# ami-iit/paper_gorbani_2025_humanoids_multi-rate-mpc-ironcub

Hardware: AMD Instinct MI355X
Metric: MPC solves/sec (whole node) + p50 single-solve latency, iRonCub paper horizon (higher is better)
Workload: dtype f64

## Files before the change

### paper_gorbani_2025_humanoids_multi-rate-mpc-ironcub_amd/csrc/vsmpc_p4.hpp

```cpp
#pragma once
#include "vsmpc_smem.hpp"

namespace vsmpc {

template <int K, int NVS>
VS_DEV double small_spd_solve(const double* __restrict__ sP, unsigned long long mask, double rhs, int lane, int& bad) {
    int idx[K];
#pragma unroll
    for (int q = 0; q < K; ++q) {
        idx[q] = __ffsll((long long)mask) - 1;
        mask &= mask - 1;
    }
    double A[K][K], d[K];
#pragma unroll
    for (int q = 0; q < K; ++q) {
        d[q] = readlane_f64(rhs, idx[q]);
#pragma unroll
        for (int c = 0; c <= q; ++c) A[q][c] = sP[idx[c] * NVS + idx[q]];
    }
    double ip[K];
#pragma unroll
    for (int j = 0; j < K; ++j) {
        bad |= !(A[j][j] > 0.0);
        ip[j] = fast_rcp(A[j][j]);
#pragma unroll
        for (int i = j + 1; i < K; ++i) {
            const double f = A[i][j] * ip[j];
            d[i] = fma(-f, d[j], d[i]);
#pragma unroll
            for (int c = j + 1; c <= i; ++c) A[i][c] = fma(-f, A[c][j], A[i][c]);
        }
    }
    double x[K], mu = 0.0;
#pragma unroll
    for (int j = K - 1; j >= 0; --j) {
        double t = d[j];
#pragma unroll
        for (int c = j + 1; c < K; ++c) t = fma(-A[c][j], x[c], t);
        x[j] = t * ip[j];
        mu = (lane == idx[j]) ? x[j] : mu;
    }
    return mu;
}

constexpr int SMALL_SOLVE_MAX = 6;
constexpr int AS_PATIENCE = 10;
constexpr int AS_MAX_ITER = 64;
template <int NVS, int K = SMALL_SOLVE_MAX>
VS_DEV double small_spd_solve_n(int k, const double* __restrict__ sP, unsigned long long mask, double rhs, int lane, int& bad) {
    if constexpr (K == 1) {
        return small_spd_solve<1, NVS>(sP, mask, rhs, lane, bad);
    } else {
        if (k == K) return small_spd_solve<K, NVS>(sP, mask, rhs, lane, bad);
        return small_spd_solve_n<NVS, K - 1>(k, sP, mask, rhs, lane, bad);
    }
}

template <class D>
VS_DEV void schur_rhs(const double* __restrict__ Lb, double* __restrict__ sSvec, int lane) {
    constexpr int PV = D::NU >> 4;
    constexpr int GR = D::NZ - 16 * (PV + 1);
    const int r = lane < D::NV ? lane : D::NV - 1;
    const double* L76 = Lb + tile_off<D>(PV + 1, PV);
    const double* L77 = Lb + tile_off<D>(PV + 1, PV + 1);
    const double* rowp = Lb + tile_off<D>(PV + (r >> 4), PV) + (r & 15) * 17;
    double sr = 0.0;
#pragma unroll
    for (int c = 0; c < D::NV; ++c) {
        const double lrc = rowp[((c >> 4) && (r >> 4)) ? D::TS + (c & 15) : (c & 15)];
        const double ellc = c < 16 ? L76[GR * 17 + c] : L77[GR * 17 + (c - 16)];
        sr = fma(c <= r ? lrc : 0.0, ellc, sr);
    }
    if (lane < D::NV) sSvec[r] = sr;
}

template <class D>
struct XTiles {
    static constexpr int NVS = D::NV + 1, NR2 = D::NV - 16;
    static constexpr int KMAX = SMALL_SOLVE_MAX;
    static constexpr int KMID = 16;
    const double* X6;
    const double* sXr;
    VS_DEV double col(int j, int r, int n) const {
        const double t = j < 16 ? X6[j * 17 + (r & 15)] : sXr[(j - 16) * NVS + r];
        return (j < 16 ? r < 16 : j < n) ? t : 0.0;
    }
    VS_DEV double pcol(int b, int r, int n) const {
        double p0 = 0.0, p1 = 0.0;
        if (b < 16) {
#pragma unroll
            for (int j = 0; j < 16; j += 2) {
                p0 = fma(col(j, r, n), X6[j * 17 + b], p0);
                p1 = fma(col(j + 1, r, n), X6[(j + 1) * 17 + b], p1);
            }
        }
#pragma unroll
        for (int a2 = 0; a2 < NR2; ++a2) p0 = fma(col(16 + a2, r, n), sXr[a2 * NVS + b], p0);
        return p0 + p1;
    }
};
template <class D>
struct XDense {
    static constexpr int NVS = D::NV + 1;
    static constexpr int KMAX = 10;
    static constexpr int KMID = 24;
    const double* sXd;
    VS_DEV double col(int j, int r, int n) const { return j < n ? sXd[j * NVS + r] : 0.0; }
    VS_DEV double pcol(int b, int r, int n) const {
        double p0 = 0.0, p1 = 0.0;
        int j = b;
        for (; j + 1 < n; j += 2) {
            p0 = fma(sXd[j * NVS + r], sXd[j * NVS + b], p0);
            p1 = fma(sXd[(j + 1) * NVS + r], sXd[(j + 1) * NVS + b], p1);
        }
        if (j < n) p0 = fma(sXd[j * NVS + r], sXd[j * NVS + b], p0);
        return p0 + p1;
    }
};

template <int KMID, int NVS>
VS_DEV double mid_spd_solve(int ka, const double* __restrict__ sP, unsigned long long Amask, double bb, int lane, bool isA,
                            int& bad) {
    int idx[KMID];
    {
        unsigned long long m = Amask;
#pragma unroll
        for (int q = 0; q < KMID; ++q) {
            idx[q] = m ? __ffsll((long long)m) - 1 : 0;
            m &= m - 1;
        }
    }
    const int rank = __popcll(Amask & ((1ull << lane) - 1ull));
    double a[KMID];
#pragma unroll
    for (int q = 0; q < KMID; ++q) a[q] = sP[idx[q] * NVS + lane];
#pragma unroll
    for (int j = 0; j < KMID; ++j) {
        if (j < ka) {
            const double piv = readlane_f64(a[j], idx[j]);
            bad |= !(piv > 0.0);
            const double ip = fast_rcp(piv);
            const double bj = readlane_f64(bb, idx[j]);
            const double f = (isA && rank > j) ? a[j] * ip : 0.0;
            bb = fma(-f, bj, bb);
#pragma unroll
            for (int c = j + 1; c < KMID; ++c) {
                if (c < ka) {
                    const double pc = readlane_f64(a[c], idx[j]);
                    a[c] = fma(-f, pc, a[c]);
                }
            }
        }
    }
    double mu = 0.0;
#pragma unroll
    for (int j = KMID - 1; j >= 0; --j) {
        if (j < ka) {
            const double xj = readlane_f64(bb, idx[j]) * fast_rcp(readlane_f64(a[j], idx[j]));
            mu = (lane == idx[j]) ? xj : mu;
            bb = (isA && rank < j) ? fma(-a[j], xj, bb) : bb;
        }
    }
    return mu;
}

template <class D, class XA>
VS_DEV void dual_active_set(const XA& xa, bool hold, int lane, double* __restrict__ sSv, double* __restrict__ sQP,
                            const double* __restrict__ sSvec, const double* __restrict__ sVprev,
                            const double* __restrict__ sCfg, double* __restrict__ sZ, int* __restrict__ sFlags,
                            unsigned long long have0 = 0ull) {
    constexpr int NVS = D::NV + 1;
    double* sP = sSv;
    double* sK = sQP;
    const int r = lane < D::NV ? lane : D::NV - 1;
    const bool valid = lane < D::NV;
    const bool fixed = valid && hold && (r >= D::NV - 4);
    const int n = hold ? D::NV - 4 : D::NV;
    const bool inN = valid && r < n;
    const double lo = fixed ? sVprev[r & 3] : sCfg[CFG_VMIN];
    const double hi = fixed ? sVprev[r & 3] : sCfg[CFG_VMAX];
    const double gtol = 1e-10 * (1.0 + sSvec[0]);
    const double vu = sZ[D::NU + r];
    int state = 0;
    double v = vu;
    int best, patience = AS_PATIENCE, status = VSMPC_STATUS_MAX_ITER, iters = 1, bad = 0;
    {
        const double tolv = 1e-12 * (1.0 + fabs(v));
        const bool vlo = inN && (v < lo - tolv);
        const bool vhi = inN && (v > hi + tolv);
        best = __popcll(__ballot(vlo || vhi));
        if (vlo || vhi) state = vlo ? -1 : 1;
    }
    unsigned long long have = have0;
    for (int it = 1; it < AS_MAX_ITER; ++it) {
        iters = it + 1;
        const bool isA = inN && state != 0;
        const unsigned long long Amask = __ballot(isA);
        unsigned long long need = Amask & ~have;
        have |= need;
        while (need) {
            const int b = __ffsll((long long)need) - 1;
            need &= need - 1;
            const double pb = xa.pcol(b, r, n);
            if (valid) sP[b * NVS + r] = pb;
        }
        double bb = isA ? vu - (state < 0 ? lo : hi) : 0.0;
        double mu = 0.0;
        const int ka = __popcll(Amask);
        if (ka == 0) {
        } else if (ka <= XA::KMAX) {
            mu = small_spd_solve_n<D::NV + 1, XA::KMAX>(ka, sP, Amask, bb, lane, bad);
        } else if (XA::KMID > 0 && ka <= XA::KMID) {
            if constexpr (XA::KMID > 0) mu = mid_spd_solve<XA::KMID, D::NV + 1>(ka, sP, Amask, bb, lane, isA, bad);
        } else {
            if (isA) {
                unsigned long long m = Amask;
                while (m) {
                    const int c = __ffsll((long long)m) - 1;
                    m &= m - 1;
                    sK[r * NVS + c] = sP[c * NVS + r];
                }
            }
            for (unsigned long long pm = Amask; pm; pm &= pm - 1) {
                const int j = __ffsll((long long)pm) - 1;
                const double piv = sK[j * NVS + j];
                bad |= !(piv > 0.0);
                const double bj = readlane_f64(bb, j);
                if (isA && lane > j) {
                    const double f = sK[r * NVS + j] * fast_rcp(piv);
                    bb -= f * bj;
                    for (unsigned long long m = pm & (pm - 1); m; m &= m - 1) {
                        const int c = __ffsll((long long)m) - 1;
                        sK[r * NVS + c] -= f * sK[j * NVS + c];
                    }
                }
            }
            for (unsigned long long pm = Amask; pm;) {
                const int j = 63 - __clzll((long long)pm);
                pm &= ~(1ull << j);
                const double xj = readlane_f64(bb, j) * fast_rcp(sK[j * NVS + j]);
                if (lane == j) mu = xj;
                if (isA && lane < j) bb -= sK[r * NVS + j] * xj;
            }
        }
        if (bad) { status = VSMPC_STATUS_NUMERICAL; break; }
        v = vu;
        for (unsigned long long m = Amask; m; m &= m - 1) {
            const int b = __ffsll((long long)m) - 1;
            const double mub = readlane_f64(mu, b);
            if (inN) v -= sP[b * NVS + r] * mub;
        }
        const double grad = -mu;
        const double tolv = 1e-12 * (1.0 + fabs(v));
        const bool isF = inN && state == 0;
        const bool vlo = isF && (v < lo - tolv);
        const bool vhi = isF && (v > hi + tolv);
        const bool rlo = isA && state == -1 && grad < -gtol;
        const bool rhi = isA && state == 1 && grad > gtol;
        const bool inf = vlo || vhi || rlo || rhi;
        const unsigned long long imask = __ballot(inf);
        const int ninf = __popcll(imask);
        if (ninf == 0) { status = VSMPC_STATUS_SOLVED; break; }
        bool pick = inf;
        if (ninf < best) { best = ninf; patience = AS_PATIENCE; }
        else if (patience > 0) { --patience; }
        else { pick = inf && (lane == 63 - __clzll(imask)); }
        if (pick) state = vlo ? -1 : (vhi ? 1 : 0);
    }
    if (valid) {
        v = fixed ? lo : (state < 0 ? lo : (state > 0 ? hi : v));
        sZ[D::NU + lane] = v;
    }
    if (lane == 0) { sFlags[1] = status; sFlags[2] = iters; }
}

template <class D>
VS_DEV void box_qp(int n_violated, bool hold, int wave) {
    using S = Smem<D>;
    extern __shared__ __attribute__((aligned(16))) double smem[];
    double* sVprev = smem + S::oVprev;
    double* sInvD = smem + S::oInvD;
    double* sZ = smem + S::oZ;
    double* sSv = smem + S::oSv;
    double* sSvec = smem + S::oSvec;
    double* sCfg = smem + S::oCfg;
    int* sFlags = reinterpret_cast<int*>(smem + S::oFlags);
    double* Lb = smem + S::oM;
    double* sXinv = smem + S::oXinv;
    double* sQP = smem + S::oQP;
    const int lane = fresh_lane(), tid = (wave << 6) | lane;
    constexpr bool DUALQP = S::DUALQP;
    constexpr int PV = D::PVT;
    constexpr int DUAL_MAX_ACTIVE = 16;
    constexpr bool DUAL3 = S::DUAL3;
    constexpr int DUAL3_MAX = 24;
    const bool few = n_violated <= (DUAL3 ? DUAL3_MAX : DUAL_MAX_ACTIVE);
    (void)sQP; (void)sXinv; (void)sInvD;
      if (few && DUALQP) {
       if constexpr (DUALQP) {
        {
            constexpr int NVS = D::NV + 1, NR2 = D::NV - 16;
            double* sXr = sQP + D::NV * NVS;
            double* sT = sQP;
            const double* X6 = sXinv + PV * D::TS;
            const double* L76 = Lb + tile_off<D>(PV + 1, PV);
            const double* L77 = Lb + tile_off<D>(PV + 1, PV + 1);
            constexpr int XT0 = 17 * NR2 <= 192 ? 16 * NR2 : 224;
            static_assert(XT0 + NR2 <= D::BLOCK && D::NV <= 32, "threads of the X77 columns");
            if (tid < 16 * NR2) {
                const int a2 = tid >> 4, j = tid & 15;
                double t0 = 0.0, t1 = 0.0;
#pragma unroll
                for (int k = 0; k < 16; k += 2) {
                    t0 = fma(L76[a2 * 17 + k], X6[k * 17 + j], t0);
                    t1 = fma(L76[a2 * 17 + k + 1], X6[(k + 1) * 17 + j], t1);
                }
                sT[a2 * 16 + j] = t0 + t1;
            } else if (tid >= XT0 && tid < XT0 + NR2) {
                const int c = tid - XT0;
                double x[NR2];
#pragma unroll
                for (int i = 0; i < NR2; ++i) {
                    double sum = 0.0;
#pragma unroll
                    for (int k = 0; k < i; ++k) sum = fma(L77[i * 17 + k], (k >= c) ? x[k] : 0.0, sum);
                    const double di = sInvD[D::NU + 16 + i];
                    x[i] = (i == c) ? di : ((i > c) ? -di * sum : 0.0);
                    sXr[i * NVS + 16 + c] = x[i];
                }
            } else if (wave == 3) {
                schur_rhs<D>(Lb, sSvec, lane);
            }
            __syncthreads();
            if (wave == 3) {
                double gm = 0.0;
#pragma unroll
                for (int c = 0; c < D::NV; ++c) gm = fmax(gm, fabs(sSvec[c]));
                if (lane == 0) sSvec[0] = gm;
            }
            if (tid < 16 * NR2) {
                const int a2 = tid >> 4, j = tid & 15;
                double t = 0.0;
#pragma unroll
                for (int b2 = 0; b2 < NR2; ++b2) t = fma(sXr[a2 * NVS + 16 + b2], sT[b2 * 16 + j], t);
                sXr[a2 * NVS + j] = -t;
            }
            __syncthreads();
        }
        static_assert(D::NU % 16 == 0 && D::NV > 16 && D::NV <= 32, "throttle block: tile aligned, two tile rows");
        const XTiles<D> xa{sXinv + PV * D::TS, sQP + D::NV * (D::NV + 1)};
        const bool all_cols = n_violated > 4;
        if (all_cols) {
            const int n = hold ? D::NV - 4 : D::NV;
            for (int e = tid; e < D::NV * D::NV; e += D::BLOCK) {
                const int b = e / D::NV, r = e - b * D::NV;
                sSv[b * (D::NV + 1) + r] = xa.pcol(b, r, n);
            }
            __syncthreads();
        }
        if (wave == 0)
            dual_active_set<D>(xa, hold, lane, sSv, sQP, sSvec, sVprev, sCfg, sZ, sFlags, all_cols ? ((1ull << D::NV) - 1ull) : 0ull);
       }
      } else if (few && DUAL3) {
       if constexpr (DUAL3) {
        constexpr int NVS = D::NV + 1, R2 = D::NV - 32;
        double* sXd = sQP + D::NV * NVS;
        double* sT0 = smem + S::oDual3T0;
        double* sT1 = smem + S::oDual3T1;
        static_assert(S::oDual3T0 == S::oQP + 2 * D::NV * NVS, "scratch tiles behind K and X");
        const double* L10 = Lb + tile_off<D>(PV + 1, PV);
        const double* L20 = Lb + tile_off<D>(PV + 2, PV);
        const double* L21 = Lb + tile_off<D>(PV + 2, PV + 1);
        const double* X0 = sXinv + PV * D::TS;
        auto xd = [&](int blk_r, int blk_c) { return sXd + (16 * blk_r) * NVS + 16 * blk_c; };
        for (int e = tid; e < D::NV * NVS; e += D::BLOCK) sXd[e] = 0.0;
        if (tid < 4 * D::NV) {
            const int i = tid >> 2, part = tid & 3;
            double sum = 0.0;
            for (int k = part; k <= i; k += 4)
                sum += Lb[lower_at<D>(D::NU + i, D::NU + k)] * Lb[lower_at<D>(D::NZ, D::NU + k)];
            sSv[tid] = sum;
        }
        __syncthreads();
        {
            const int g = lane >> 4, n = lane & 15;
            auto a_tile = [&](const double* T, int ks) { return T[n * 17 + 4 * ks + g]; };
            auto b_tile = [&](const double* T, int ks) { return T[(4 * ks + g) * 17 + n]; };
            auto a_x2 = [&](int ks) {
                const double v = sT1[n * 17 + 4 * ks + g];
                return (n < R2 && 4 * ks + g < R2) ? v : 0.0;
            };
            const d4 zero = d4{0.0, 0.0, 0.0, 0.0};
            if (wave == 0) {
                d4 t10 = zero, x10 = zero, t20 = zero, x20 = zero;
#pragma unroll
                for (int ks = 0; ks < 4; ++ks) t10 = __builtin_amdgcn_mfma_f64_16x16x4f64(a_tile(L10, ks), b_tile(X0, ks), t10, 0, 0, 0);
#pragma unroll
                for (int ks = 0; ks < 4; ++ks) t20 = __builtin_amdgcn_mfma_f64_16x16x4f64(a_tile(L20, ks), b_tile(X0, ks), t20, 0, 0, 0);
#pragma unroll
                for (int ks = 0; ks < 4; ++ks) x10 = __builtin_amdgcn_mfma_f64_16x16x4f64(a_tile(sT0, ks), t10[ks], x10, 0, 0, 0);
#pragma unroll
                for (int r = 0; r < 4; ++r) { x10[r] = -x10[r]; xd(1, 0)[(g + 4 * r) * NVS + n] = x10[r]; }
#pragma unroll
                for (int ks = 0; ks < 4; ++ks) t20 = __builtin_amdgcn_mfma_f64_16x16x4f64(a_tile(L21, ks), x10[ks], t20, 0, 0, 0);
#pragma unroll
                for (int ks = 0; ks < 4; ++ks) x20 = __builtin_amdgcn_mfma_f64_16x16x4f64(a_x2(ks), t20[ks], x20, 0, 0, 0);
#pragma unroll
                for (int r = 0; r < 4; ++r)
                    if (g + 4 * r < R2) xd(2, 0)[(g + 4 * r) * NVS + n] = -x20[r];
            } else if (wave == 1) {
                d4 t21 = zero, x21 = zero;
#pragma unroll
                for (int ks = 0; ks < 4; ++ks) t21 = __builtin_amdgcn_mfma_f64_16x16x4f64(a_tile(L21, ks), b_tile(sT0, ks), t21, 0, 0, 0);
#pragma unroll
                for (int ks = 0; ks < 4; ++ks) x21 = __builtin_amdgcn_mfma_f64_16x16x4f64(a_x2(ks), t21[ks], x21, 0, 0, 0);
#pragma unroll
                for (int r = 0; r < 4; ++r)
                    if (g + 4 * r < R2) xd(2, 1)[(g + 4 * r) * NVS + n] = -x21[r];
            } else if (wave == 2) {
#pragma unroll
                for (int r = 0; r < 4; ++r) {
                    const int i = g + 4 * r;
                    const double x0 = X0[i * 17 + n], x1 = sT0[i * 17 + n], x2 = sT1[i * 17 + n];
                    if (n <= i) {
                        xd(0, 0)[i * NVS + n] = x0;
                        xd(1, 1)[i * NVS + n] = x1;
                        if (i < R2) xd(2, 2)[i * NVS + n] = x2;
                    }
                }
            } else {
                if (lane < D::NV) sSvec[lane] = (sSv[4 * lane] + sSv[4 * lane + 1]) + (sSv[4 * lane + 2] + sSv[4 * lane + 3]);
                double gm = 0.0;
                for (int c = 0; c < D::NV; ++c) gm = fmax(gm, fabs(sSvec[c]));
                if (lane == 0) sSvec[0] = gm;
            }
        }
        __syncthreads();
        {
            static_assert(D::NV <= 48, "three tile rows");
            const int n = hold ? D::NV - 4 : D::NV;
            const int g = lane >> 4, m = lane & 15;
#pragma unroll 1
            for (int t = wave; t < 6; t += D::NWAVES) {
                const int ta = t < 1 ? 0 : (t < 3 ? 1 : 2), tb = t - ta * (ta + 1) / 2;
                const int ca = 16 * ta + m, cb = 16 * tb + m;
                double xa_[12], xb_[12];
#pragma unroll
                for (int ks = 0; ks < 12; ++ks) {
                    const int j = 4 * ks + g;
                    const double va = sXd[j * NVS + ca], vb = sXd[j * NVS + cb];
                    xa_[ks] = (j < n && ca < D::NV) ? va : 0.0;
                    xb_[ks] = (j < n && cb < D::NV) ? vb : 0.0;
                }
                d4 c0 = d4{0.0, 0.0, 0.0, 0.0}, c1 = d4{0.0, 0.0, 0.0, 0.0};
#pragma unroll
                for (int ks = 0; ks < 12; ks += 2) {
                    c0 = __builtin_amdgcn_mfma_f64_16x16x4f64(xa_[ks], xb_[ks], c0, 0, 0, 0);
                    c1 = __builtin_amdgcn_mfma_f64_16x16x4f64(xa_[ks + 1], xb_[ks + 1], c1, 0, 0, 0);
                }
#pragma unroll
                for (int r = 0; r < 4; ++r) {
                    const int i = 16 * ta + g + 4 * r;
                    const double pv = c0[r] + c1[r];
                    if (i < D::NV && cb < D::NV) {
                        sSv[cb * NVS + i] = pv;
                        sSv[i * NVS + cb] = pv;
                    }
                }
            }
        }
        __syncthreads();
        if (wave == 0) {
            const XDense<D> xa{sXd};
            dual_active_set<D>(xa, hold, lane, sSv, sQP, sSvec, sVprev, sCfg, sZ, sFlags, ~0ull);
        }
       }
      } else {
        for (int e = tid; e < D::NV * D::NV; e += D::BLOCK) {
            const int r = e / D::NV, c = e % D::NV;
            const int kmax = r < c ? r : c;
            double sum = 0.0;
            for (int k = 0; k <= kmax; ++k)
                sum += Lb[lower_at<D>(D::NU + r, D::NU + k)] * Lb[lower_at<D>(D::NU + c, D::NU + k)];
            sSv[r * (D::NV + 1) + c] = sum;
        }
        if (tid < D::NV) {
            double sum = 0.0;
            for (int k = 0; k <= tid; ++k)
                sum += Lb[lower_at<D>(D::NU + tid, D::NU + k)] * Lb[lower_at<D>(D::NZ, D::NU + k)];
            sSvec[tid] = sum;
        }
        __syncthreads();

        if (wave == 0) {
            const int r = lane < D::NV ? lane : D::NV - 1;
            const bool valid = lane < D::NV;
            double row[D::NV];
#pragma unroll
            for (int c = 0; c < D::NV; ++c) row[c] = sSv[r * (D::NV + 1) + c];
            const double svr = sSvec[r];
            const bool fixed = valid && hold && (r >= D::NV - 4);
            const double lo = fixed ? sVprev[r & 3] : sCfg[CFG_VMIN];
            const double hi = fixed ? sVprev[r & 3] : sCfg[CFG_VMAX];
            int state = fixed ? -1 : 0;
            double gmax = fabs(svr);
#pragma unroll
            for (int o = 32; o > 0; o >>= 1) gmax = fmax(gmax, __shfl_xor(gmax, o));
            const double gtol = 1e-10 * (1.0 + gmax);
            double v = sZ[D::NU + r];
            int best, patience = AS_PATIENCE, status = VSMPC_STATUS_MAX_ITER, iters = 1;
            {
                const double tolv = 1e-12 * (1.0 + fabs(v));
                const bool vlo = valid && state == 0 && (v < lo - tolv);
                const bool vhi = valid && state == 0 && (v > hi + tolv);
                best = __popcll(__ballot(vlo || vhi));
                if (vlo || vhi) state = vlo ? -1 : 1;
            }
            for (int it = 1; it < AS_MAX_ITER; ++it) {
                iters = it + 1;
                const bool isF = valid && state == 0;
                const unsigned long long Fmask = __ballot(isF);
                const double vb = isF ? 0.0 : (state < 0 ? lo : hi);
                double a[D::NV];
                double b = isF ? -svr : vb;
#pragma unroll
                for (int c = 0; c < D::NV; ++c) {
                    const bool cF = (Fmask >> c) & 1ull;
                    const double vbc = readlane_f64(vb, c);
                    if (isF && !cF) b -= row[c] * vbc;
                    a[c] = (isF && cF) ? row[c] : ((c == r && !isF) ? 1.0 : 0.0);
                }
                int bad = 0;
                const int nfree = __popcll(Fmask);
                if (nfree >= 1 && nfree <= SMALL_SOLVE_MAX) {
                    const double vf = small_spd_solve_n<D::NV + 1>(nfree, sSv, Fmask, b, lane, bad);
                    v = isF ? vf : vb;
                } else {
#pragma unroll
                for (int j = 0; j < D::NV; ++j) {
                    if ((Fmask >> j) & 1ull) {
                        const double piv = readlane_f64(a[j], j);
                        bad |= !(piv > 0.0);
                        const double f = (lane > j) ? a[j] * fast_rcp(piv) : 0.0;
                        const double bj = readlane_f64(b, j);
                        b -= f * bj;
#pragma unroll
                        for (int c = j + 1; c < D::NV; ++c) {
                            const double pc = readlane_f64(a[c], j);
                            a[c] -= f * pc;
                        }
                    }
                }
                v = vb;
#pragma unroll
                for (int j = D::NV - 1; j >= 0; --j) {
                    if ((Fmask >> j) & 1ull) {
                        const double xj = readlane_f64(b, j) * fast_rcp(readlane_f64(a[j], j));
                        if (lane == j) v = xj;
                        if (lane < j) b -= a[j] * xj;
                    }
                }
                }
                if (bad) { status = VSMPC_STATUS_NUMERICAL; break; }
                double grad = svr;
#pragma unroll
                for (int c = 0; c < D::NV; ++c) grad += row[c] * readlane_f64(v, c);
                const double tolv = 1e-12 * (1.0 + fabs(v));
                const bool vlo = isF && (v < lo - tolv);
                const bool vhi = isF && (v > hi + tolv);
                const bool rlo = valid && state == -1 && !fixed && grad < -gtol;
                const bool rhi = valid && state == 1 && !fixed && grad > gtol;
                const bool inf = vlo || vhi || rlo || rhi;
                const unsigned long long imask = __ballot(inf);
                const int ninf = __popcll(imask);
                if (ninf == 0) { status = VSMPC_STATUS_SOLVED; break; }
                bool pick = inf;
                if (ninf < best) { best = ninf; patience = AS_PATIENCE; }
                else if (patience > 0) { --patience; }
                else { pick = inf && (lane == 63 - __clzll(imask)); }
                if (pick) state = vlo ? -1 : (vhi ? 1 : 0);
            }
            if (valid) {
                v = state < 0 ? lo : (state > 0 ? hi : v);
                sZ[D::NU + lane] = v;
            }
            if (lane == 0) { sFlags[1] = status; sFlags[2] = iters; }
        }
      }
}

}
```

### paper_gorbani_2025_humanoids_multi-rate-mpc-ironcub_amd/csrc/vsmpc_smem.hpp

```cpp
#pragma once
#include <type_traits>

#include "vsmpc_device.hpp"

namespace vsmpc {

typedef double d4 __attribute__((ext_vector_type(4)));

template <class D, bool PIPE = false>
__device__ constexpr TileTab<D, PIPE> kTileTab{};
template <class D>
__device__ constexpr NactTab<D> kNactTab{};
template <class D>
__device__ constexpr TilePack<D> kTilePack{};

template <int I, int N, class F>
VS_DEV void static_for(F&& f) {
    if constexpr (I < N) {
        f(std::integral_constant<int, I>{});
        static_for<I + 1, N>(f);
    }
}

VS_DEV int fresh_lane() {
    unsigned m = ~0u;
    asm volatile("" : "+s"(m));
    return int(__builtin_amdgcn_mbcnt_hi(m, __builtin_amdgcn_mbcnt_lo(m, 0u)));
}

template <class D>
struct Smem {
    static constexpr bool DUALQP = D::NT - 2 == D::PVT && D::NU % 16 == 0 && D::NV >= 20 && D::NV <= 32;
    static constexpr int oIn = 0;
    static constexpr int oA = oIn + ((D::NIN + 3) & ~3);
    static constexpr int oBj = oA + NX * NX;
    static constexpr int oBt = oBj + NX * NJ;
    static constexpr int oC = oBt + NX * NTH;
    static constexpr int oVprev = oC + 28;
    static constexpr int oInvD = oVprev + 4;
    static constexpr int oW = oInvD + D::NP;
    static constexpr int oZ = oW + D::NP;
    static constexpr int oSvec = oZ + D::NP;
    static constexpr int oV = oSvec + D::NV;
    static constexpr int oDt = oV + D::NV;
    static constexpr int oCfg = oDt + MAX_STAGES;
    static constexpr int oFlags = oCfg + CFG_SIZE;
    static constexpr int oQR = (oFlags + 4 + 3) & ~3;
    static constexpr int QR_V = 0, QR_BETA = 48, QR_GY = 56, QR_NS = 62, QR_ISW = 64, QR_A = 72, QR_SIZE = 128;
    static constexpr int NXT = D::PVT + 1;
    static constexpr int oXinv = (oQR + QR_SIZE + 3) & ~3;
    static constexpr int oR = oXinv + NXT * D::TS;
    static constexpr int YROWS = 36;
    static constexpr int oY = oR;
    static constexpr int sizeY = YROWS * D::YS;
    static constexpr int oM = oR;
    static constexpr int sizeM = D::L_TILES * D::TS;
    static constexpr int NVS = D::NV + 1;
    static constexpr int oSv = oR;
    static constexpr bool DUAL3 = !DUALQP && D::NT - 3 == D::PVT && D::NU % 16 == 0 && D::NV > 32 && D::NV <= 48;
    static constexpr int oQP = oSv + D::NV * NVS;
    static constexpr int sizeQP = DUALQP ? D::NV * NVS + (D::NV - 16) * NVS : (DUAL3 ? 2 * D::NV * NVS + 2 * D::TS : 0);
    static constexpr int oDual3T0 = oQP + 2 * D::NV * NVS;
    static constexpr int oDual3T1 = oDual3T0 + D::TS;
    static constexpr int oU = DUAL3 ? oR : oQP + sizeQP;
    static constexpr int oX = oU + D::NWAVES * D::NP;
    static constexpr int oF = oX + D::NXS;
    static constexpr int endScratch = (oF + NX * D::N > oQP + sizeQP) ? oF + NX * D::N : oQP + sizeQP;
    static_assert(endScratch <= oR + D::CORNER_TILE0 * D::TS, "P4..P6 scratch must not reach the corner tiles");
    static constexpr int NJROW = D::NV + NTH + 1;
    static constexpr int oJetT = oXinv;
    static constexpr int oGA = oJetT + NJROW * D::N;
    static constexpr int oSH = oGA + 6 * D::N;
    static constexpr int oSRb = oSH + 2 * D::NJPAIR * 9;
    static constexpr int oSW3 = oSRb + 2 * (D::NV + 1) * D::HC * 3;
    static constexpr int oSAc = oSW3 + (D::STRUCT_LONG ? 0 : 2 * (D::NV + 1) * (D::N - 1) * 3);
    static constexpr int AC_SHORT = D::STRUCT_LONG ? D::NV - NTH : 0;
    static constexpr int AC_NSH = D::STRUCT_LONG ? D::NS : 0;
    VS_HD static constexpr int ac_first(int cr) { return cr < AC_SHORT ? AC_NSH : 0; }
    VS_HD static constexpr int ac_off(int cr) {
        return 4 * (cr * (D::N - 1) - (cr < AC_SHORT ? cr : AC_SHORT) * AC_NSH);
    }
    static constexpr int sizeAc = ac_off(D::NV + 1);
    static constexpr int oSRefC = oSAc + sizeAc;
    static constexpr int sizeZero = 3 * D::N > 12 * D::NREF ? 3 * D::N : 12 * D::NREF;
    static constexpr int oSZero = D::STRUCT_LONG ? oW : oSRefC + 12 * D::NREF;
    static_assert(!D::STRUCT_LONG || sizeZero <= 2 * D::NP, "zeros fit the w and z vectors");
    static constexpr int endP1s = D::STRUCT_LONG ? oSRefC + 12 * D::NREF : oSZero + sizeZero;
    static constexpr int oNextDiag = oM + sizeM;
    static constexpr int total_syrk = oR + (sizeY > sizeM ? sizeY : sizeM);
    static constexpr int total_struct = D::STRUCT_P1 ? (endP1s > oNextDiag + D::TS ? endP1s : oNextDiag + D::TS) : total_syrk;
    static constexpr int total = total_syrk;
    static constexpr size_t bytes = size_t(total) * sizeof(double);
    static constexpr size_t bytes_struct = size_t(total_struct) * sizeof(double);
    static_assert(bytes <= 160 * 1024 && bytes_struct <= 160 * 1024, "LDS budget of one CU");
    static_assert(D::WG_PER_CU < 2 || (bytes <= 80 * 1024 && bytes_struct <= 80 * 1024), "two workgroups per CU");
};

template <class D>
VS_HD constexpr int tile_off_c(int i, int j) {
    return (j < D::PVT ? (j & 1) * D::RING_A + (i - j)
                       : D::CORNER_TILE0 + (i - D::PVT) * (i - D::PVT + 1) / 2 + (j - D::PVT)) * D::TS;
}
template <class D>
VS_DEV int tile_off(int i, int j) { return tile_off_c<D>(i, j); }

template <class D>
VS_DEV int lower_at(int gr, int gc) {
    return tile_off<D>(gr >> 4, gc >> 4) + (gr & 15) * 17 + (gc & 15);
}

}
```

### paper_gorbani_2025_humanoids_multi-rate-mpc-ironcub_amd/csrc/vsmpc_solve_body.inc

```
#define VS_STAMP(i)                                                                         \
    do {                                                                                    \
        if constexpr (STAMPS) {                                                             \
            unsigned long long* st_ = late_args()->stamps;                                  \
            if (tid == 0 && st_ != nullptr) st_[size_t(blockIdx.x) * 16 + (i)] = __builtin_amdgcn_s_memtime(); \
        }                                                                                   \
    } while (0)
    unsigned long long t_acc[6] = {0, 0, 0, 0, 0, 0};
    unsigned long long t_mark = 0, stamp_t1 = 0, rt0 = 0;
    if constexpr (STAMPS) rt0 = __builtin_amdgcn_s_memrealtime();
#define VS_TIC()                                                     \
    do {                                                             \
        if constexpr (STAMPS) t_mark = __builtin_amdgcn_s_memtime(); \
    } while (0)
#define VS_TOC(i)                                                          \
    do {                                                                   \
        if constexpr (STAMPS) {                                            \
            const unsigned long long t_now = __builtin_amdgcn_s_memtime(); \
            t_acc[i] += t_now - t_mark;                                    \
            t_mark = t_now;                                                \
        }                                                                  \
    } while (0)
    using S = Smem<D>;
    constexpr bool FUSED_DISPATCH = FORM == 1;
    constexpr bool PIPE = FORM == 1;
// ... 402 lines not shown
                    syrk_fixed(std::integral_constant<int, pg.nks[g]>{}, std::integral_constant<int, pg.nact[g]>{});
                    VS_TOC(2);
                    __syncthreads();
                }
            });
        }
        VS_TIC();
    }
    if constexpr (!FUSED_DISPATCH) VS_STAMP(2);
    VS_REFRESH_IDS();
    if constexpr (D::WG_PER_CU == 1) pin_tiles_agpr<TPW>(acc);

    constexpr int PVT = D::PVT;
    const int crow = (lane >> 4) * 17 + (lane & 15);
    const int lrow = (lane & 15) * 17 + (lane >> 4);
    double* dbgM = STAMPS ? late_args()->dbgM : nullptr;
    double* dbgL = STAMPS ? late_args()->dbgL : nullptr;
    double* dbgLi = dbgL != nullptr ? dbgL + size_t(inst) * D::NP * D::NP : nullptr;
    if (STAMPS && !FUSED_DISPATCH && dbgM != nullptr) {
#pragma unroll
        for (int q = 0; q < TPW; ++q) {
            if (kTileTab<D, PIPE>.forms(q * D::NWAVES + wave, wave)) {
                const int ti_q = kTileTab<D, PIPE>.ti[q * D::NWAVES + wave], tj_q = kTileTab<D, PIPE>.tj[q * D::NWAVES + wave];
                d4 tmp = acc[q];
                if (ti_q == tj_q || ti_q >= PVT) {
#pragma unroll
                    for (int r = 0; r < 4; ++r)
                        tmp[r] += input_cost_term<D>(sCfg, smem + S::oQR + S::QR_GY, sVprev, 16 * ti_q + (lane >> 4) + 4 * r,
                                                     16 * tj_q + (lane & 15));
                }
#pragma unroll
                for (int r = 0; r < 4; ++r) {
                    const int gr = 16 * ti_q + (lane >> 4) + 4 * r, gc = 16 * tj_q + (lane & 15);
                    if (gc <= gr) dbgM[size_t(inst) * D::NP * D::NP + size_t(gr) * D::NP + gc] = tmp[r];
                }
            }
        }
    }
    if constexpr (!FUSED_DISPATCH) VS_STAMP(3);
    VS_REFRESH_IDS();
    if constexpr (!FUSED_DISPATCH)
    switch (wave) {
        case 0: cholesky_wave<D, TPW, 0, STAMPS, PIPE>(sCfg, acc, Lb, sInvD, smem + S::oQR + S::QR_GY, sVprev, sFlags, sXinv, sW, dbgLi, lane, crow, lrow, sZ); break;
        case 1: cholesky_wave<D, TPW, 1, STAMPS, PIPE>(sCfg, acc, Lb, sInvD, smem + S::oQR + S::QR_GY, sVprev, sFlags, sXinv, sW, dbgLi, lane, crow, lrow, sZ); break;
        case 2: cholesky_wave<D, TPW, 2, STAMPS, PIPE>(sCfg, acc, Lb, sInvD, smem + S::oQR + S::QR_GY, sVprev, sFlags, sXinv, sW, dbgLi, lane, crow, lrow, sZ); break;
        default: cholesky_wave<D, TPW, 3, STAMPS, PIPE>(sCfg, acc, Lb, sInvD, smem + S::oQR + S::QR_GY, sVprev, sFlags, sXinv, sW, dbgLi, lane, crow, lrow, sZ); break;
    }
    static_assert(D::NWAVES == 4, "wave-specialised phases are instantiated for four wavefronts");
    if (STAMPS && dbgLi != nullptr) {
        if constexpr (!FUSED_DISPATCH) {
#pragma unroll
            for (int q = 0; q < TPW; ++q) {
                const int ti_q = kTileTab<D, PIPE>.ti[q * D::NWAVES + wave], tj_q = kTileTab<D, PIPE>.tj[q * D::NWAVES + wave];
                if (kTileTab<D, PIPE>.holds(q * D::NWAVES + wave, wave) && tj_q < PVT && ti_q > tj_q) {
#pragma unroll
                    for (int r = 0; r < 4; ++r)
                        dbgLi[size_t(16 * ti_q + (lane >> 4) + 4 * r) * D::NP + 16 * tj_q + (lane & 15)] = acc[q][r];
                }
            }
        }
        for (int e = tid; e < (D::NP - 16 * PVT) * (D::NP - 16 * PVT); e += D::BLOCK) {
            const int gr = 16 * PVT + e / (D::NP - 16 * PVT), gc = 16 * PVT + e % (D::NP - 16 * PVT);
            if (gc <= gr) dbgLi[size_t(gr) * D::NP + gc] = Lb[lower_at<D>(gr, gc)];
        }
    }

    VS_STAMP(4);
    VS_REFRESH_IDS();
    if constexpr (D::WG_PER_CU == 1) pin_tiles_agpr<TPW>(acc);
    const bool hold = sIn[VSMPC_IN_HOLD] != 0.0;
    constexpr int PV = D::PVT;
    auto init_corner_rhs = [&]() {
        if (tid >= 16 * PV && tid < D::NP) sW[tid] = tid < D::NZ ? -Lb[lower_at<D>(D::NZ, tid)] : 0.0;
    };
    init_corner_rhs();
    if (tid < D::NP) sZ[tid] = (hold && tid >= D::NZ - 4 && tid < D::NZ) ? sVprev[tid - (D::NZ - 4)] : 0.0;
    __syncthreads();

    auto sweep_tile = [&](int p, bool prescribed) {
        if (wave == 0) {
            const int j = lane & 15;
            const int gj = 16 * p + j;
            const double* Tpp = Lb + tile_off<D>(p, p) + j;
            double colv[16];
#pragma unroll
            for (int k = 0; k < 16; ++k) {
                const double t = Tpp[k * 17];
                colv[k] = k >= j ? t : 0.0;
            }
            double w = sW[gj];
            const bool fix = (gj >= D::NZ) || (gj >= D::NU && (prescribed || (hold && gj >= D::NZ - 4)));
            const double inv_eff = fix ? 0.0 : sInvD[gj];
            const double zadd = (fix && gj < D::NZ) ? sZ[gj] : 0.0;
            double z = 0.0;
#pragma unroll
            for (int k = 15; k >= 0; --k) {
                const double zk = readlane_f64(fma(w, inv_eff, zadd), k);
                z = (j == k) ? zk : z;
                w = fma(-colv[k], zk, w);
            }
            if (lane < 16) sZ[gj] = z;
        }
        __syncthreads();
        if (p > PV) {
            if (tid >= 16 * PV && tid < 16 * p) {
                const double* T = Lb + tile_off<D>(p, tid >> 4) + (tid & 15);
                const double* zp = sZ + 16 * p;
                double a2 = 0.0;
#pragma unroll
                for (int k = 0; k < 16; ++k) a2 += T[k * 17] * zp[k];
                sW[tid] -= a2;
            }
            __syncthreads();
        }
    };

    constexpr bool DUALQP = S::DUALQP;
    if constexpr (DUALQP) {
        constexpr int PL = D::NT - 1, KL = D::NZ - 16 * PL;
        static_assert(KL == D::NV - 16 && KL >= 4, "pins live in the last tile row");
        const double* X6 = sXinv + PV * D::TS;
        const double* L76 = Lb + tile_off<D>(PL, PV);
        const double* L77 = Lb + tile_off<D>(PL, PL);
        if (wave == 0) {
            const int j = lane & 15;
            const int gj = 16 * PL + j;
            const double* Tpp = L77 + j;
            double colv[KL], l76[KL], x6[16];
#pragma unroll
            for (int k = 0; k < KL; ++k) {
                const double t = Tpp[k * 17];
                colv[k] = k >= j ? t : 0.0;
                l76[k] = L76[k * 17 + j];
            }
#pragma unroll
            for (int i = 0; i < 16; ++i) x6[i] = X6[i * 17 + j];
            double w = sW[gj];
            double w6 = sW[16 * PV + j];
            const bool fix = (j >= KL) || (hold && j >= KL - 4);
            const double inv_eff = fix ? 0.0 : sInvD[gj];
            const double zadd = (fix && j < KL) ? sZ[gj] : 0.0;
            double z = 0.0;
#pragma unroll
            for (int k = KL - 1; k >= 0; --k) {
                const double zk = readlane_f64(fma(w, inv_eff, zadd), k);
                z = (j == k) ? zk : z;
                w = fma(-colv[k], zk, w);
                w6 = fma(-l76[k], zk, w6);
            }
            double z6 = 0.0;
#pragma unroll
            for (int i = 0; i < 16; ++i) z6 = fma(x6[i], readlane_f64(w6, i), z6);
            if (lane < 16) { sZ[gj] = z; sZ[16 * PV + j] = z6; }
        }
    } else if constexpr (S::DUAL3) {
        static_assert(D::NT - 1 == PV + 2, "three throttle tile rows");
        double x2[16];
        const double* L22d = Lb + tile_off_c<D>(PV + 2, PV + 2);
        const double* inv2 = sInvD + D::NU + 32;
        if (wave == 1) tile_inverse_rows<0, 8>(L22d, inv2, x2, lane);
        sweep_tile(PV + 2, false);
        auto sweep_tile_x = [&](int p, const double* Xp) {
            if (wave == 0) {
                const int j = lane & 15;
                double z0 = 0.0, z1 = 0.0;
#pragma unroll
                for (int k = 0; k < 16; k += 2) {
                    z0 = fma(Xp[k * 17 + j], sW[16 * p + k], z0);
                    z1 = fma(Xp[(k + 1) * 17 + j], sW[16 * p + k + 1], z1);
                }
                if (lane < 16) sZ[16 * p + j] = z0 + z1;
            }
            __syncthreads();
            if (p > PV) {
                if (tid >= 16 * PV && tid < 16 * p) {
                    const double* T = Lb + tile_off<D>(p, tid >> 4) + (tid & 15);
                    const double* zp = sZ + 16 * p;
                    double a2 = 0.0;
#pragma unroll
                    for (int k = 0; k < 16; ++k) a2 += T[k * 17] * zp[k];
                    sW[tid] -= a2;
                }
                __syncthreads();
            }
        };
        if (wave == 1) tile_inverse_rows<8, 13>(L22d, inv2, x2, lane);
        sweep_tile_x(PV + 1, smem + S::oDual3T0);
        if (wave == 1) {
            tile_inverse_rows<13, 16>(L22d, inv2, x2, lane);
            if (lane < 16) {
#pragma unroll
                for (int i = 0; i < 16; ++i) smem[S::oDual3T1 + i * 17 + lane] = x2[i];
            }
        }
        sweep_tile_x(PV, sXinv + PV * D::TS);
    } else {
#pragma unroll 1
        for (int p = D::NT - 1; p >= PV; --p) sweep_tile(p, false);
    }
    if (wave == 0) {
        const bool valid = lane < D::NV;
        const double v = sZ[D::NU + (valid ? lane : 0)];
        const bool fixed = hold && lane >= D::NV - 4;
        const double tolv = 1e-12 * (1.0 + fabs(v));
        const bool viol = valid && !fixed && (v < sCfg[CFG_VMIN] - tolv || v > sCfg[CFG_VMAX] + tolv);
        const unsigned long long vm = __ballot(viol);
        if (lane == 0) { sFlags[3] = __popcll(vm); sFlags[1] = VSMPC_STATUS_SOLVED; sFlags[2] = 1; }
    }
    __syncthreads();
    const bool need_qp = sFlags[3] != 0;
    VS_STAMP(5);
    VS_REFRESH_IDS();

    if (need_qp) {
        box_qp<D>(sFlags[3], hold, wave);
        __syncthreads();
        VS_STAMP(6);
        VS_REFRESH_IDS();
        if constexpr (D::NU % 16 != 0) {
            init_corner_rhs();
            __syncthreads();
#pragma unroll 1
            for (int p = D::NT - 1; p >= PV; --p) sweep_tile(p, true);
        }
    } else {
        VS_STAMP(6);
    }
    switch (wave) {
        case 0:
            if constexpr (PIPE) p5_wave0_jets<D>(smem, lane);
            else backsub_wave<D, TPW, 0, PIPE>(acc, sW, sZ, sXinv, sU, lane);
            break;
        case 1: backsub_wave<D, TPW, 1, PIPE>(acc, sW, sZ, sXinv, sU, lane); break;
        case 2: backsub_wave<D, TPW, 2, PIPE>(acc, sW, sZ, sXinv, sU, lane); break;
        default: backsub_wave<D, TPW, 3, PIPE>(acc, sW, sZ, sXinv, sU, lane); break;
    }
    if (tid < D::NV) sV[tid] = sZ[D::NU + tid];
    __syncthreads();

    VS_STAMP(7);
    VS_REFRESH_IDS();
#ifdef VS_DIAG_P6
    for (int i = 0; i < 4; ++i) t_acc[i] = 0;
    VS_TIC();
#define VS_P6_TOC(i) VS_TOC(i)
#else
#define VS_P6_TOC(i) do { } while (0)
#endif
    const SolveArgs* ka = late_args();
    double* xout = ka->xout;
    double* fmout = ka->fmout;
    int* status_out = ka->status_out;
    int* iters_out = ka->iters_out;
    double u8[8] = {0.0, 0.0, 0.0, 0.0, 0.0, 0.0, 0.0, 0.0};
    constexpr int JX_SPLIT = PIPE ? 3 : NJC;
    if (PIPE && wave == 3 && lane < D::HC) joint_expand<D, NJC, JX_SPLIT>(smem + S::oQR, sZ + NJC * lane, u8);
    {
        constexpr int ROWS = PIPE ? 6 : NX;
        constexpr int NE = ROWS * D::N, RND = (NE + D::BLOCK - 1) / D::BLOCK;
#pragma unroll
        for (int rd = 0; rd < RND; ++rd) {
            const int e0 = tid + rd * D::BLOCK, ec = e0 < NE ? e0 : NE - 1;
            const int k = ec / ROWS, rr = ec - k * ROWS;
            const int r = PIPE ? (rr < 3 ? 3 + rr : 6 + rr) : rr;
            const int e = NX * k + r;
            const int jb = joint_block_of_stage<D>(k);
            const int tb = throttle_block_of_stage<D>(k);
            const int vq = tb == 0 ? D::NV - 4 : 4 * (tb - 1);
            double f = sC[r];
#pragma unroll
            for (int c = 0; c < NJC; ++c) f += sBj[r * NJ + c] * sZ[NJC * jb + c];
#pragma unroll
            for (int c = 0; c < NTH; ++c) f += sBt[r * NTH + c] * sV[vq + c];
            if (e0 < NE) sF[e] = f;
        }
    }
    __syncthreads();
    VS_P6_TOC(0);
    {
        constexpr int CHK = D::N > 20 ? 9 : 6, NCH = (D::N + CHK - 1) / CHK;
        double jT = 0.0, jTd = 0.0, jon = 0.0, ja = 0.0, jb = 0.0;
        double Sk[9], hh[3] = {0.0, 0.0, 0.0};
        double cm0 = 0.0, cm1 = 0.0, cm2 = 0.0, cce = 0.0, cx = 0.0, cee = 0.0;
        const int hr0m = (lane & 1) ? 9 : 3;
        const int cg = lane / 3, cr = lane - 3 * cg;
        const int cxr = (cg ? 6 : 0) + cr, chr0 = cg ? 9 : 3, cer = (cg ? 23 : 20) + cr;
        constexpr bool JETS_EARLY = PIPE;
        constexpr int JOFF = JETS_EARLY ? 0 : 1;
        if (!JETS_EARLY && wave == 0 && lane < NTH) {
            jon = sA[(12 + lane) * NX + 16 + lane]; ja = sA[(16 + lane) * NX + 12 + lane]; jb = sA[(16 + lane) * NX + 16 + lane];
            jT = sIn[VSMPC_IN_X0 + 12 + lane]; jTd = sIn[VSMPC_IN_X0 + 16 + lane];
            sX[12 + lane] = jT;
            sX[16 + lane] = jTd;
        }
        if (wave == 1 && lane < 2) {
#pragma unroll
            for (int r = 0; r < 3; ++r) {
                hh[r] = sIn[VSMPC_IN_X0 + hr0m + r];
                sX[hr0m + r] = hh[r];
#pragma unroll
                for (int c = 0; c < 3; ++c) Sk[3 * r + c] = sA[(hr0m + r) * NX + hr0m + c];
            }
        }
        if (wave == 2 && lane < 6) {
            cm0 = sA[cxr * NX + chr0]; cm1 = sA[cxr * NX + chr0 + 1]; cm2 = sA[cxr * NX + chr0 + 2];
            cce = sC[cer];
            cx = sIn[VSMPC_IN_X0 + cxr]; cee = sIn[VSMPC_IN_X0 + cer];
            sX[cxr] = cx;
            sX[cer] = cee;
        }
        static_assert(D::NUO <= D::NWAVES * D::NP, "joint increments fit the partial-sum array");
        if (wave == 3 && lane < D::HC) {
            if constexpr (PIPE) joint_expand<D, JX_SPLIT, 0>(smem + S::oQR, sZ + NJC * lane, u8);
            else joint_expand<D>(smem + S::oQR, sZ + NJC * lane, u8);
#pragma unroll
            for (int i = 0; i < 8; ++i) sU[NJ * lane + i] = u8[i];
        }
        if (wave == 3 && xout != nullptr) {
            double2* xo = reinterpret_cast<double2*>(xout + size_t(inst) * D::NVAR);
            for (int i = lane; i < D::NUO / 2; i += 64) xo[D::NXS / 2 + i] = make_double2(sU[2 * i], sU[2 * i + 1]);
            if (lane < D::NV / 2) {
                const int e = 2 * lane, b = e >> 2, c = e & 3;
                const int q = b == 0 ? D::NV - 4 + c : 4 * (b - 1) + c;
                xo[(D::NXS + D::NUO) / 2 + lane] = make_double2(sV[q], sV[q + 1]);
            }
        }

        static_for<0, NCH + 1 + JOFF>([&](auto scst) __attribute__((always_inline)) {
            constexpr int st = decltype(scst)::value;
            if constexpr (!JETS_EARLY && st < NCH) {
                if (wave == 0 && lane < NTH) {
                    constexpr int k0 = st * CHK;
                    double fa[CHK], fb[CHK], dtk[CHK];
#pragma unroll
                    for (int u = 0; u < CHK; ++u) {
                        const int k = (k0 + u < D::N) ? k0 + u : D::N - 1;
                        fa[u] = sF[NX * k + 12 + lane];
                        fb[u] = sF[NX * k + 16 + lane];
                        dtk[u] = sDt[k];
                    }
#pragma unroll
                    for (int u = 0; u < CHK; ++u) {
                        const double dT = fma(jon, jTd, fa[u]);
                        const double dTd = fma(ja, jT, fma(jb, jTd, fb[u]));
                        jT = fma(dtk[u], dT, jT);
                        jTd = fma(dtk[u], dTd, jTd);
                        if (k0 + u < D::N) {
                            sX[NX * (k0 + u + 1) + 12 + lane] = jT;
                            sX[NX * (k0 + u + 1) + 16 + lane] = jTd;
                        }
                    }
                }
            }
            if constexpr (PIPE && st == 1) {
                if (wave == 3 && fmout != nullptr && lane < VSMPC_FM_SIZE) {
                    double v;
                    if (lane < 8) v = sU[lane];
                    else if (lane < 12) v = sV[D::NV - 4 + (lane - 8)];
                    else if (lane < 16) v = Jet::throttle_of_v(sV[D::NV - 4 + (lane - 12)]);
                    else if (lane < 20) v = sX[NX + 12 + (lane - 16)];
                    else v = sX[NX + 16 + (lane - 20)];
                    fmout[size_t(inst) * VSMPC_FM_SIZE + lane] = v;
                }
            }
            if constexpr (st >= JOFF && st - JOFF < NCH) {
                if (wave == 1) {
                    constexpr int k0 = (st - JOFF) * CHK;
                    constexpr int kn = k0 + CHK < D::N ? CHK : D::N - k0;
// ... 101 lines not shown
```

Before: 7.500 million.

## Overlap dual QP setup with the back-sweep and pre-load violated P columns

Moves the dual QP setup (the X76 partial product, the X77 inverse columns, the Schur rhs and its max-norm) out of box_qp and into the idle waves during the final tile sweep, so the work runs alongside the wave-0 sweep. This removes a block-wide barrier and a serial phase from the QP path. It also records the initially violated mask in a new flag slot and, when 2-4 bounds are violated, has waves 0-3 each precompute one P column in parallel before the single-wave active-set loop. Optional QP timing instrumentation is added behind a macro. The setup work now runs on every solve even when no QP is needed, which adds cost on those solves.

After: 7.681 million (median of 6 runs). +2.4%, better.

```diff
diff --git a/paper_gorbani_2025_humanoids_multi-rate-mpc-ironcub_amd/csrc/vsmpc_p4.hpp b/paper_gorbani_2025_humanoids_multi-rate-mpc-ironcub_amd/csrc/vsmpc_p4.hpp
--- a/paper_gorbani_2025_humanoids_multi-rate-mpc-ironcub_amd/csrc/vsmpc_p4.hpp
+++ b/paper_gorbani_2025_humanoids_multi-rate-mpc-ironcub_amd/csrc/vsmpc_p4.hpp
@@ -2,6 +2,21 @@
 #include "vsmpc_smem.hpp"
 
 namespace vsmpc {
+
+#ifdef VS_DIAG_QP
+#define VS_QP_TIC() do { if (qt != nullptr) qt_mark = __builtin_amdgcn_s_memtime(); } while (0)
+#define VS_QP_TOC(i)                                                   \
+    do {                                                               \
+        if (qt != nullptr) {                                           \
+            const unsigned long long qt_now = __builtin_amdgcn_s_memtime(); \
+            qt[i] += qt_now - qt_mark;                                 \
+            qt_mark = qt_now;                                          \
+        }                                                              \
+    } while (0)
+#else
+#define VS_QP_TIC() do { } while (0)
+#define VS_QP_TOC(i) do { } while (0)
+#endif
 
 template <int K, int NVS>
 VS_DEV double small_spd_solve(const double* __restrict__ sP, unsigned long long mask, double rhs, int lane, int& bad) {
@@ -164,11 +179,76 @@
     return mu;
 }
 
+VS_DEV void wave_lds_sync() {
+    __builtin_amdgcn_fence(__ATOMIC_RELEASE, "wavefront");
+    __builtin_amdgcn_wave_barrier();
+    __builtin_amdgcn_fence(__ATOMIC_ACQUIRE, "wavefront");
+}
+
+template <class D>
+VS_DEV void dual_setup_beside_sweep(int wave, int lane) {
+    using S = Smem<D>;
+    extern __shared__ __attribute__((aligned(16))) double smem[];
+    constexpr int PV = D::PVT, NVS = D::NV + 1, NR2 = D::NV - 16;
+    static_assert(S::DUALQP && NR2 >= 1 && NR2 <= 16, "two throttle tile rows");
+    double* Lb = smem + S::oM;
+    double* sQP = smem + S::oQP;
+    double* sXr = sQP + D::NV * NVS;
+    double* sT = sQP;
+    if (wave == 1) {
+        const double* X6 = smem + S::oXinv + PV * D::TS;
+        const double* L76 = Lb + tile_off<D>(PV + 1, PV);
+        constexpr int RND = (16 * NR2 + 63) / 64;
+#pragma unroll
+        for (int rd = 0; rd < RND; ++rd) {
+            const int e = lane + 64 * rd;
+            if (e < 16 * NR2) {
+                const int a2 = e >> 4, j = e & 15;
+                double t0 = 0.0, t1 = 0.0;
+#pragma unroll
+                for (int k = 0; k < 16; k += 2) {
+                    t0 = fma(L76[a2 * 17 + k], X6[k * 17 + j], t0);
+                    t1 = fma(L76[a2 * 17 + k + 1], X6[(k + 1) * 17 + j], t1);
+                }
+                sT[a2 * 16 + j] = t0 + t1;
+            }
+        }
+    } else if (wave == 2) {
+        const double* sInvD = smem + S::oInvD;
+        const double* L77 = Lb + tile_off<D>(PV + 1, PV + 1);
+        if (lane < NR2) {
+            const int c = lane;
+            double x[NR2];
+#pragma unroll
+            for (int i = 0; i < NR2; ++i) {
+                double sum = 0.0;
+#pragma unroll
+                for (int k = 0; k < i; ++k) sum = fma(L77[i * 17 + k], (k >= c) ? x[k] : 0.0, sum);
+                const double di = sInvD[D::NU + 16 + i];
+                x[i] = (i == c) ? di : ((i > c) ? -di * sum : 0.0);
+                sXr[i * NVS + 16 + c] = x[i];
+            }
+        }
+    } else {
+        double* sSvec = smem + S::oSvec;
+        schur_rhs<D>(Lb, sSvec, lane);
+        wave_lds_sync();
+        double gm = 0.0;
+#pragma unroll
+        for (int c = 0; c < D::NV; ++c) gm = fmax(gm, fabs(sSvec[c]));
+        wave_lds_sync();
+        if (lane == 0) sSvec[0] = gm;
+    }
+}
+
 template <class D, class XA>
 VS_DEV void dual_active_set(const XA& xa, bool hold, int lane, double* __restrict__ sSv, double* __restrict__ sQP,
                             const double* __restrict__ sSvec, const double* __restrict__ sVprev,
                             const double* __restrict__ sCfg, double* __restrict__ sZ, int* __restrict__ sFlags,
-                            unsigned long long have0 = 0ull) {
+                            unsigned long long have0 = 0ull, unsigned long long* qt = nullptr) {
+    unsigned long long qt_mark = 0;
+    (void)qt; (void)qt_mark;
+    VS_QP_TIC();
     constexpr int NVS = D::NV + 1;
     double* sP = sSv;
     double* sK = sQP;
@@ -204,6 +284,7 @@
             const double pb = xa.pcol(b, r, n);
             if (valid) sP[b * NVS + r] = pb;
         }
+        VS_QP_TOC(1);
         double bb = isA ? vu - (state < 0 ? lo : hi) : 0.0;
         double mu = 0.0;
         const int ka = __popcll(Amask);
@@ -243,6 +324,7 @@
                 if (isA && lane < j) bb -= sK[r * NVS + j] * xj;
             }
         }
+        VS_QP_TOC(2);
         if (bad) { status = VSMPC_STATUS_NUMERICAL; break; }
         v = vu;
         for (unsigned long long m = Amask; m; m &= m - 1) {
@@ -266,7 +348,9 @@
         else if (patience > 0) { --patience; }
         else { pick = inf && (lane == 63 - __clzll(imask)); }
         if (pick) state = vlo ? -1 : (vhi ? 1 : 0);
-    }
+        VS_QP_TOC(3);
+    }
+    VS_QP_TOC(3);
     if (valid) {
         v = fixed ? lo : (state < 0 ? lo : (state > 0 ? hi : v));
         sZ[D::NU + lane] = v;
@@ -275,7 +359,10 @@
 }
 
 template <class D>
-VS_DEV void box_qp(int n_violated, bool hold, int wave) {
+VS_DEV void box_qp(int n_violated, bool hold, int wave, unsigned long long* qt = nullptr) {
+    unsigned long long qt_mark = 0;
+    (void)qt; (void)qt_mark;
+    VS_QP_TIC();
     using S = Smem<D>;
     extern __shared__ __attribute__((aligned(16))) double smem[];
     double* sVprev = smem + S::oVprev;
@@ -301,43 +388,8 @@
         {
             constexpr int NVS = D::NV + 1, NR2 = D::NV - 16;
             double* sXr = sQP + D::NV * NVS;
-            double* sT = sQP;
-            const double* X6 = sXinv + PV * D::TS;
-            const double* L76 = Lb + tile_off<D>(PV + 1, PV);
-            const double* L77 = Lb + tile_off<D>(PV + 1, PV + 1);
-            constexpr int XT0 = 17 * NR2 <= 192 ? 16 * NR2 : 224;
-            static_assert(XT0 + NR2 <= D::BLOCK && D::NV <= 32, "threads of the X77 columns");
-            if (tid < 16 * NR2) {
-                const int a2 = tid >> 4, j = tid & 15;
-                double t0 = 0.0, t1 = 0.0;
-#pragma unroll
-                for (int k = 0; k < 16; k += 2) {
-                    t0 = fma(L76[a2 * 17 + k], X6[k * 17 + j], t0);
-                    t1 = fma(L76[a2 * 17 + k + 1], X6[(k + 1) * 17 + j], t1);
-                }
-                sT[a2 * 16 + j] = t0 + t1;
-            } else if (tid >= XT0 && tid < XT0 + NR2) {
-                const int c = tid - XT0;
-                double x[NR2];
-#pragma unroll
-                for (int i = 0; i < NR2; ++i) {
-                    double sum = 0.0;
-#pragma unroll
-                    for (int k = 0; k < i; ++k) sum = fma(L77[i * 17 + k], (k >= c) ? x[k] : 0.0, sum);
-                    const double di = sInvD[D::NU + 16 + i];
-                    x[i] = (i == c) ? di : ((i > c) ? -di * sum : 0.0);
-                    sXr[i * NVS + 16 + c] = x[i];
-                }
-            } else if (wave == 3) {
-                schur_rhs<D>(Lb, sSvec, lane);
-            }
-            __syncthreads();
-            if (wave == 3) {
-                double gm = 0.0;
-#pragma unroll
-                for (int c = 0; c < D::NV; ++c) gm = fmax(gm, fabs(sSvec[c]));
-                if (lane == 0) sSvec[0] = gm;
-            }
+            const double* sT = sQP;
+            static_assert(16 * NR2 <= D::BLOCK, "one entry of X76 per thread");
             if (tid < 16 * NR2) {
                 const int a2 = tid >> 4, j = tid & 15;
                 double t = 0.0;
@@ -347,9 +399,11 @@
             }
             __syncthreads();
         }
+        VS_QP_TOC(0);
         static_assert(D::NU % 16 == 0 && D::NV > 16 && D::NV <= 32, "throttle block: tile aligned, two tile rows");
         const XTiles<D> xa{sXinv + PV * D::TS, sQP + D::NV * (D::NV + 1)};
         const bool all_cols = n_violated > 4;
+        const bool first_cols = !all_cols && n_violated >= 2;
         if (all_cols) {
             const int n = hold ? D::NV - 4 : D::NV;
             for (int e = tid; e < D::NV * D::NV; e += D::BLOCK) {
@@ -357,9 +411,23 @@
                 sSv[b * (D::NV + 1) + r] = xa.pcol(b, r, n);
             }
             __syncthreads();
-        }
+        } else if (first_cols) {
+            const int n = hold ? D::NV - 4 : D::NV;
+            unsigned m = unsigned(sFlags[4]);
+            for (int q = 0; q < wave; ++q) m &= m - 1;
+            if (m) {
+                const int b = __ffs(int(m)) - 1;
+                const int r = lane < D::NV ? lane : D::NV - 1;
+                const double pb = xa.pcol(b, r, n);
+                if (lane < D::NV) sSv[b * (D::NV + 1) + r] = pb;
+            }
+            __syncthreads();
+        }
+        VS_QP_TOC(1);
         if (wave == 0)
-            dual_active_set<D>(xa, hold, lane, sSv, sQP, sSvec, sVprev, sCfg, sZ, sFlags, all_cols ? ((1ull << D::NV) - 1ull) : 0ull);
+            dual_active_set<D>(xa, hold, lane, sSv, sQP, sSvec, sVprev, sCfg, sZ, sFlags,
+                               all_cols ? ((1ull << D::NV) - 1ull) : (first_cols ? (unsigned long long)unsigned(sFlags[4]) : 0ull),
+                               qt);
        }
       } else if (few && DUAL3) {
        if constexpr (DUAL3) {
@@ -589,4 +657,7 @@
       }
 }
 
-}
+#undef VS_QP_TIC
+#undef VS_QP_TOC
+
+}
diff --git a/paper_gorbani_2025_humanoids_multi-rate-mpc-ironcub_amd/csrc/vsmpc_smem.hpp b/paper_gorbani_2025_humanoids_multi-rate-mpc-ironcub_amd/csrc/vsmpc_smem.hpp
--- a/paper_gorbani_2025_humanoids_multi-rate-mpc-ironcub_amd/csrc/vsmpc_smem.hpp
+++ b/paper_gorbani_2025_humanoids_multi-rate-mpc-ironcub_amd/csrc/vsmpc_smem.hpp
@@ -45,6 +45,8 @@
     static constexpr int oDt = oV + D::NV;
     static constexpr int oCfg = oDt + MAX_STAGES;
     static constexpr int oFlags = oCfg + CFG_SIZE;
+    static constexpr int NFLAGS = 5;
+    static_assert(NFLAGS * sizeof(int) <= 4 * sizeof(double), "the int flags fit their four doubles (oQR follows)");
     static constexpr int oQR = (oFlags + 4 + 3) & ~3;
     static constexpr int QR_V = 0, QR_BETA = 48, QR_GY = 56, QR_NS = 62, QR_ISW = 64, QR_A = 72, QR_SIZE = 128;
     static constexpr int NXT = D::PVT + 1;
diff --git a/paper_gorbani_2025_humanoids_multi-rate-mpc-ironcub_amd/csrc/vsmpc_solve_body.inc b/paper_gorbani_2025_humanoids_multi-rate-mpc-ironcub_amd/csrc/vsmpc_solve_body.inc
--- a/paper_gorbani_2025_humanoids_multi-rate-mpc-ironcub_amd/csrc/vsmpc_solve_body.inc
+++ b/paper_gorbani_2025_humanoids_multi-rate-mpc-ironcub_amd/csrc/vsmpc_solve_body.inc
@@ -578,6 +578,8 @@
 #pragma unroll
             for (int i = 0; i < 16; ++i) z6 = fma(x6[i], readlane_f64(w6, i), z6);
             if (lane < 16) { sZ[gj] = z; sZ[16 * PV + j] = z6; }
+        } else {
+            dual_setup_beside_sweep<D>(wave, lane);
         }
     } else if constexpr (S::DUAL3) {
         static_assert(D::NT - 1 == PV + 2, "three throttle tile rows");
@@ -632,14 +634,24 @@
         const bool viol = valid && !fixed && (v < sCfg[CFG_VMIN] - tolv || v > sCfg[CFG_VMAX] + tolv);
         const unsigned long long vm = __ballot(viol);
         if (lane == 0) { sFlags[3] = __popcll(vm); sFlags[1] = VSMPC_STATUS_SOLVED; sFlags[2] = 1; }
+        if constexpr (DUALQP) {
+            if (lane == 0) sFlags[4] = int(unsigned(vm));
+        }
     }
     __syncthreads();
     const bool need_qp = sFlags[3] != 0;
     VS_STAMP(5);
     VS_REFRESH_IDS();
 
+#ifdef VS_DIAG_QP
+    for (int i = 0; i < 4; ++i) t_acc[i] = 0;
+#endif
     if (need_qp) {
+#ifdef VS_DIAG_QP
+        box_qp<D>(sFlags[3], hold, wave, STAMPS ? t_acc : nullptr);
+#else
         box_qp<D>(sFlags[3], hold, wave);
+#endif
         __syncthreads();
         VS_STAMP(6);
         VS_REFRESH_IDS();
```
